# AI-ON/Few-Shot-Music-Generation

Hardware: AMD Instinct MI355X
Metric: episodes/s (LSTM-baseline train step, synthetic vocab=10k seq_len=128 5-way/5-shot h=512) (higher is better)
Workload: dtype f32 (bf16x3-split products, fp32 accumulate)

## Files before the change

### few-shot-music-generation_amd/csrc/api_comm.hip

```cpp
#include "fsmg_model.h"

using namespace fsmg;
using namespace fsmg_host;

namespace fsmg_host {

struct Rccl {
    typedef struct { char internal[128]; } UniqueId;
    int (*GetUniqueId)(UniqueId*) = nullptr;
    int (*CommInitRank)(void**, int, UniqueId, int) = nullptr;
    int (*CommDestroy)(void*) = nullptr;
    int (*AllReduce)(const void*, void*, size_t, int, int, void*, hipStream_t) = nullptr;
    int (*Broadcast)(const void*, void*, size_t, int, int, void*, hipStream_t) = nullptr;
    int (*GroupStart)() = nullptr; int (*GroupEnd)() = nullptr;
    const char* (*GetErrorString)(int) = nullptr;
    std::string why;
    bool ok = false;
    Rccl() {
        static const char* names[] = {"librccl.so", "librccl.so.1", "/opt/rocm/lib/librccl.so.1", "/opt/rocm/lib/librccl.so"};
        void* lib = nullptr;
        for (const char* name : names) if (!lib) lib = dlopen(name, RTLD_NOW | RTLD_NOLOAD | RTLD_GLOBAL);
        for (const char* name : names) if (!lib) lib = dlopen(name, RTLD_NOW | RTLD_GLOBAL);
        if (!lib) { why = "librccl.so not found (dlopen)"; return; }
        GetUniqueId = (int (*)(UniqueId*))dlsym(lib, "ncclGetUniqueId");
        CommInitRank = (int (*)(void**, int, UniqueId, int))dlsym(lib, "ncclCommInitRank");
        CommDestroy = (int (*)(void*))dlsym(lib, "ncclCommDestroy");
        AllReduce = (int (*)(const void*, void*, size_t, int, int, void*, hipStream_t))dlsym(lib, "ncclAllReduce");
        Broadcast = (int (*)(const void*, void*, size_t, int, int, void*, hipStream_t))dlsym(lib, "ncclBroadcast");
        GroupStart = (int (*)())dlsym(lib, "ncclGroupStart");
        GroupEnd = (int (*)())dlsym(lib, "ncclGroupEnd");
        GetErrorString = (const char* (*)(int))dlsym(lib, "ncclGetErrorString");
        ok = GetUniqueId && CommInitRank && CommDestroy && AllReduce && Broadcast && GroupStart && GroupEnd && GetErrorString;
        if (!ok) why = "librccl.so lacks an expected symbol";
    }
};
inline Rccl& rccl() { static Rccl r; return r; }
constexpr int NCCL_FLOAT = 7, NCCL_SUM = 0, NCCL_CHAR = 0;
#define NCCLCK(h, call)                                                                                   \
    do {                                                                                                  \
        const int e_ = (call);                                                                            \
        if (e_ != 0) return fail(h, FSMG_ERR_HIP, std::string(#call) + ": " + rccl().GetErrorString(e_)); \
    } while (0)

void comm_destroy(fsmg_model* h) {
    if (h->comm && h->own_comm && rccl().ok) rccl().CommDestroy(h->comm);
    if (h->ev_comm) hipEventDestroy(h->ev_comm);
    if (h->comm_stream) hipStreamDestroy(h->comm_stream);
    h->comm = nullptr; h->ev_comm = nullptr; h->comm_stream = nullptr;
}

int exchange_gradients(fsmg_model* h) {
    Rccl& r = rccl();
    HIPCK(h, hipStreamWaitEvent(h->comm_stream, h->ev_bucket[0], 0));
    NCCLCK(h, r.AllReduce(h->G + h->off_w, h->G + h->off_w, (size_t)(h->n_flat - h->off_w), NCCL_FLOAT, NCCL_SUM, h->comm, h->comm_stream));
    HIPCK(h, hipStreamWaitEvent(h->comm_stream, h->ev_bucket[1], 0));
    NCCLCK(h, r.GroupStart());
    NCCLCK(h, r.AllReduce(h->G, h->G, (size_t)h->off_w, NCCL_FLOAT, NCCL_SUM, h->comm, h->comm_stream));
    NCCLCK(h, r.AllReduce(h->G + h->n_flat, h->G + h->n_flat, (size_t)FSMG_GRAD_TAIL, NCCL_FLOAT, NCCL_SUM, h->comm, h->comm_stream));
    NCCLCK(h, r.GroupEnd());
    HIPCK(h, hipEventRecord(h->ev_comm, h->comm_stream));
    HIPCK(h, hipStreamWaitEvent(h->stream, h->ev_comm, 0));
    return FSMG_OK;
}

}

extern "C" {

static int comm_prepare(fsmg_handle h) {
    if (!rccl().ok) return fail(h, FSMG_ERR_STATE, "RCCL is not available: " + rccl().why);
    BEGIN_CALL(h);
    if (!h->comm_stream) HIPCK(h, hipStreamCreateWithFlags(&h->comm_stream, hipStreamNonBlocking));
    if (!h->ev_comm) HIPCK(h, hipEventCreateWithFlags(&h->ev_comm, hipEventDisableTiming));
    return FSMG_OK;
}

int fsmg_comm_unique_id(char id[FSMG_COMM_ID_BYTES]) {
    if (!id) return FSMG_ERR_INVALID;
    if (!rccl().ok) return fail(nullptr, FSMG_ERR_STATE, "RCCL is not available: " + rccl().why);
    Rccl::UniqueId u;
    const int e = rccl().GetUniqueId(&u);
    if (e != 0) return fail(nullptr, FSMG_ERR_HIP, std::string("ncclGetUniqueId: ") + rccl().GetErrorString(e));
    std::memcpy(id, u.internal, FSMG_COMM_ID_BYTES);
    return FSMG_OK;
}

int fsmg_comm_init(fsmg_handle h, const char id[FSMG_COMM_ID_BYTES], int32_t world_size, int32_t rank) {
    if (!h || !id || world_size < 1 || rank < 0 || rank >= world_size) return FSMG_ERR_INVALID;
    if (h->comm) return fail(h, FSMG_ERR_STATE, "a communicator is already attached");
    int rc = comm_prepare(h);
    if (rc != FSMG_OK) return rc;
    Rccl::UniqueId u;
    std::memcpy(u.internal, id, FSMG_COMM_ID_BYTES);
    void* c = nullptr;
    NCCLCK(h, rccl().CommInitRank(&c, world_size, u, rank));
    h->comm = c; h->own_comm = true; h->world = world_size; h->rank = rank;
    drop_graphs(h);
    return FSMG_OK;
}

int fsmg_comm_attach(fsmg_handle h, void* nccl_comm, int32_t world_size, int32_t rank) {
    if (!h || !nccl_comm || world_size < 1 || rank < 0 || rank >= world_size) return FSMG_ERR_INVALID;
    if (h->comm) return fail(h, FSMG_ERR_STATE, "a communicator is already attached");
    int rc = comm_prepare(h);
    if (rc != FSMG_OK) return rc;
    h->comm = nccl_comm; h->own_comm = false; h->world = world_size; h->rank = rank;
// ... 32 lines not shown
```

### few-shot-music-generation_amd/csrc/api_debug.hip

```cpp
#include "fsmg_model.h"

using namespace fsmg;
using namespace fsmg_host;


extern "C" {

int fsmg_debug_clock_begin(fsmg_handle h, int32_t microseconds) {
    if (!h || microseconds <= 0 || microseconds > 1000000) return FSMG_ERR_INVALID;
    BEGIN_CALL(h, true);
    if (!h->probe) HIPCK(h, hipStreamCreateWithFlags(&h->probe, hipStreamNonBlocking));
    if (!h->d_probe) HIPCK(h, hipMalloc((void**)&h->d_probe, 64));
    HIPCK(h, hipMemsetAsync(h->d_probe, 0, 64, h->probe));
    HIPCK(h, launch_clock_probe(h->probe, (long long)microseconds * 100, h->d_probe));
    return FSMG_OK;
}
int fsmg_debug_clock_end(fsmg_handle h, float* ghz) {
    if (!h || !ghz) return FSMG_ERR_INVALID;
    if (!h->probe || !h->d_probe) return fail(h, FSMG_ERR_STATE, "fsmg_debug_clock_end without fsmg_debug_clock_begin");
    BEGIN_CALL(h, true);
    unsigned long long v[2] = {0, 0};
    HIPCK(h, hipStreamSynchronize(h->probe));
    HIPCK(h, hipMemcpy(v, h->d_probe, sizeof(v), hipMemcpyDeviceToHost));
    *ghz = v[1] ? (float)((double)v[0] / (double)v[1] * 0.1) : 0.0f;
    return FSMG_OK;
}

int fsmg_debug_dims(fsmg_handle h, int32_t dims[5]) {
    if (!h || !dims) return FSMG_ERR_INVALID;
    dims[0] = h->Ep; dims[1] = h->Hp; dims[2] = h->V1p; dims[3] = h->lastB; dims[4] = h->T;
    return FSMG_OK;
}

int fsmg_debug_read(fsmg_handle h, const char* what, float* host, int64_t count) {
    if (!h || !what || !host || count <= 0) return FSMG_ERR_INVALID;
    const int upd_state = h->upd_deferred ? 2 : h->upd_pending ? 1 : 0;
    BEGIN_CALL(h, !std::strcmp(what, "upd_defer"));
    const int64_t B = h->lastB, T = h->T, Hp = h->Hp, G4 = h->G4, rows = T * B;
    const float* src = nullptr; int64_t cap = 0;
    auto layer_of = [&](const char* prefix) -> int {
        const size_t n = std::strlen(prefix);
        if (std::strncmp(what, prefix, n) != 0) return -1;
        const int l = std::atoi(what + n);
        return (l >= 0 && l < h->L && std::strlen(what) > n) ? l : -1;
    };
    int l;
    if (!std::strcmp(what, "aux_tries")) { host[0] = (float)h->aux_tries; return FSMG_OK; }
    if (!std::strcmp(what, "fused_softmax")) { host[0] = h->fused_softmax ? 1.0f : 0.0f; if (count > 1) host[1] = h->fs_call ? 1.0f : 0.0f; return FSMG_OK; }
    if (!std::strcmp(what, "upd_defer")) {
        const float v[4] = {h->upd_defer ? 1.0f : 0.0f, (float)upd_state, (float)h->n_upd_placed, (float)h->n_upd_settled};
        for (int64_t i = 0; i < count && i < 4; ++i) host[i] = v[i];
        return FSMG_OK;
    }
    if (!std::strcmp(what, "xcd_bx3")) { host[0] = h->xcd_bx3 ? 1.0f : 0.0f; return FSMG_OK; }
    if (!std::strcmp(what, "gemm_kinds")) {
        for (int64_t i = 0; i < count && i < 4; ++i) host[i] = (float)h->gemm_kinds[i];
        return FSMG_OK;
    }
    if (!std::strcmp(what, "xov_selfcheck")) {
        const float v[3] = {(float)h->xov_selfcheck_runs, (float)h->xov_passes, (float)h->xov_selfcheck_every};
        for (int64_t i = 0; i < count && i < 3; ++i) host[i] = v[i];
        return FSMG_OK;
    }
    if (!std::strcmp(what, "xcd_partitioned")) {
        host[0] = h->xov ? 1.0f : 0.0f;
        if (count > 1) { const int b = h->lastB > 0 ? h->lastB : 45, rpx = lstm_xcd16_packed_rows(b, h->Hp); host[1] = (h->xov && rpx > 0) ? (float)xov_first_free(b, h->Hp) : 8.0f; }
        if (count > 2) host[2] = h->xov_last ? 1.0f : 0.0f;
        return FSMG_OK;
    }
    if (!std::strncmp(what, "adapted:", 8)) {
        if (!h->have_adapted) return fail(h, FSMG_ERR_STATE, "no adapted parameters kept: fsmg_debug_set(\"keep_adapted\", 1), then a MAML-style call");
        return download_tensor(h, h->P_adapted, what + 8, host, count);
    }
    if (!std::strcmp(what, "logits")) { src = h->logits; cap = rows * h->V1p; }
    else if (!std::strcmp(what, "dlogits")) { src = dlogits_buf(h); cap = rows * h->V1p; }
    else if (!std::strcmp(what, "lse")) { src = h->lse; cap = rows; }
    else if (!std::strcmp(what, "ce")) { src = h->ce; cap = rows; }
    else if (!std::strcmp(what, "row_weight")) { src = h->roww; cap = h->last_mask_groups > 0 ? rows : 0; }
    else if (!std::strcmp(what, "n_valid")) {
        if (count > h->last_mask_groups) return fail(h, FSMG_ERR_SIZE, "debug read larger than the buffer");
        std::vector<int> nv((size_t)count);
        HIPCK(h, hipStreamSynchronize(h->stream));
        HIPCK(h, hipMemcpy(nv.data(), h->d_nvalid, sizeof(int) * count, hipMemcpyDeviceToHost));
        for (int64_t i = 0; i < count; ++i) host[i] = (float)nv[(size_t)i];
// ... 88 lines not shown
```

### few-shot-music-generation_amd/csrc/api_forward.hip

```cpp
#include "fsmg_model.h"

using namespace fsmg;
using namespace fsmg_host;

namespace fsmg_host {

int stage_tokens(fsmg_model* h, const int32_t* support, int n_sup, const int32_t* query, int n_qry, int on_device) {
    const size_t T = h->T;
    if (on_device && h->eager_call) {
        h->cur_sup = support; h->cur_qry = query;
        return FSMG_OK;
    }
    const hipMemcpyKind kind = on_device ? hipMemcpyDeviceToDevice : hipMemcpyHostToDevice;
    if (n_sup > 0) HIPCK(h, hipMemcpyAsync(h->d_tok, support, sizeof(int) * n_sup * T, kind, h->stream));
    if (n_qry > 0) HIPCK(h, hipMemcpyAsync(h->d_tok + n_sup * T, query, sizeof(int) * n_qry * T, kind, h->stream));
    h->cur_sup = h->d_tok; h->cur_qry = h->d_tok + n_sup * T;
    return FSMG_OK;
}

int stage_lengths(fsmg_model* h, const int32_t* support_len, int n_sup, const int32_t* query_len, int n_qry, int on_device) {
    const hipMemcpyKind kind = on_device ? hipMemcpyDeviceToDevice : hipMemcpyHostToDevice;
    if (n_sup > 0) HIPCK(h, hipMemcpyAsync(h->d_len, support_len, sizeof(int) * n_sup, kind, h->stream));
    if (n_qry > 0) HIPCK(h, hipMemcpyAsync(h->d_len + n_sup, query_len, sizeof(int) * n_qry, kind, h->stream));
    h->cur_len = h->d_len;
// ... 95 lines not shown
}

int forward(fsmg_model* h, int B, int rows_per_group, int ngroups, float* loss_out, bool want_dlogits, int head) {
    ScopedRange rng_(want_dlogits ? "fsmg.forward(train)" : head == HEAD_LOGITS ? "fsmg.forward(score)" : head == HEAD_NONE ? "fsmg.forward(cache)" : "fsmg.forward(eval)");
    const int T = h->T, Hp = h->Hp, G4 = h->G4;
    const int64_t rows = (int64_t)T * B;
    const Lane mainl = main_lane(h);
    hipStream_t s = h->stream;
    const bool ov = head == HEAD_LOSS && use_overlap(h);
    const bool xcd = use_xcd(h, B);
    const bool chain1 = !xcd && h->persist && !h->force_fwd_rt && lstm_fwd_chain_supported(B, Hp);
    const bool chain_rt = !xcd && h->persist && !chain1 && lstm_fwd_chain_rt_supported(B, Hp);
    const bool chain = chain1 || chain_rt;
    if (!xcd && h->cs_stale) return fail(h, FSMG_ERR_STATE, "internal: forward pass on the column-split kernels with stale fragment copies of K_h (ensure_cs not called)");
    const int nch_ov = ov ? ((chain || xcd) ? h->nchunk_persist : h->nchunk) : 1;
    GemmArgs ghead = logits_args(h, B, 0, T);
    h->fs_call = false;
    if (want_dlogits && h->fused_softmax && !ov && h->bx3 && h->inplace_dlogits && h->Hsc != nullptr && mainl.lds_pad == 0) {
        h->fs_call = true;
        h->fs_call = use_h_gemm(h, OP_XC, OP_XC, dw_args(h, B), mainl);
    }
    if (h->fs_call) fused_softmax_args(h, ghead);
    const bool xov = h->xov_call && (h->xov_parts & 1) && xcd && want_dlogits && !ov && xov_fits(ghead);
    const int xfree = xov_first_free(B, Hp);
    const int rpx = xov ? lstm_xcd16_packed_rows(B, Hp) : 0;
    if (xov) xov_gate(h, ghead, B);
    for (int l = 0; l < h->L; ++l) {
        const size_t Bp16 = (size_t)(B + 15) / 16 * 16;
        const bool top = l == h->L - 1;
        FillBatch fills(h);
        GEMMCK(fills.add(h->Hs[l], 0u, (long long)B * Hp));
        GEMMCK(fills.add(h->Cs[l], 0u, (long long)B * Hp));
        if (!xcd) GEMMCK(fills.add(h->HF[l], 0u, (long long)Bp16 * Hp));
        {
            ScopedTimer tm(h, "gemm_zx");
            GemmArgs g{};
            if (l == 0) { g.A = h->P + h->off_emb; g.lda = h->Ep; g.gather = h->X; g.K = h->Ep; }
            else { g.A = h->Hs[l - 1] + (size_t)B * Hp; g.lda = Hp; g.K = Hp; }
            g.B = h->P + h->off_kx[l]; g.ldb = G4;
            g.C = h->Z[l]; g.ldc = G4; g.M = (int)rows; g.N = G4;
            g.bias = h->P + h->off_b[l]; g.ksplit = 1;
            GEMMCK(gemm(h, mainl, OP_KC, OP_XC, g));
        }
        auto chain_fills = [&]() -> int {
            if (chain)
                GEMMCK(fills.add(h->HF[l] + Bp16 * Hp, 0xFFFFFFFFu, (long long)T * Bp16 * Hp));
            if (xcd) {
                GEMMCK(fills.add(h->tickets, 0u, (long long)8 * fsmg_model::TICKET_LAUNCHES));
                h->ticket_next = 0;
                const int rpx_l = xov && top ? rpx : 0;
                const long long step_f = lstm_xcd_hx_floats(B, 0, Hp, h->xcd_bx3, rpx_l);
                const long long used_f = step_f / lstm_xcd_slices(Hp) * lstm_xcd_used_slices(B, rpx_l, Hp);
                GEMMCK(fills.add(h->HX, 0u, step_f));
                GEMMCK(fills.add_strided(h->HX + step_f, 0xFFFFFFFFu, used_f, step_f, T));
                if (xov && top) {
                    GEMMCK(fills.add(h->xov_ctl, 0u, 4 + gemm_items(ghead)));
                    GEMMCK(fills.add(h->xov_prog, 0u, T));
                }
            }
            return fills.flush();
        };
        const bool place = l == 0 && h->upd_deferred && xov && top && xfree >= 1 && xfree <= 7;
        if (place) GEMMCK(place_deferred_half(h, xfree));
        GEMMCK(chain_fills());
        if (l == 0 && !place) GEMMCK(settle_pending(h));
        if (xov && top) {
            HIPCK(h, hipEventRecord(h->ev_fork, s));
            HIPCK(h, hipStreamWaitEvent(h->aux, h->ev_fork, 0));
            GEMMCK(gemm_restricted(h, h->aux, OP_KC, OP_XC, ghead, xfree, h->xov_ctl));
            HIPCK(h, hipEventRecord(h->ev_join, h->aux));
        }
        const int nch = nch_ov;
        for (int c = 0; c < nch; ++c) {
            const int t0 = chunk_begin(h, c, nch);
            const int t1 = chunk_begin(h, c + 1, nch);
            if (xcd) {
                ScopedTimer tm(h, "lstm_fwd");
                LstmFwdXcdArgs a{};
                a.rpx = (xov && top) ? rpx : 0; a.progress = (xov && top) ? h->xov_prog : nullptr; a.Hp = Hp;
                a.progress_every = h->xov_pub; a.bx3 = h->xcd_bx3 ? 1 : 0;
                a.variant = h->xcd_variant >= 0 ? h->xcd_variant : lstm_xcd_default_variant(B, true, Hp, a.rpx, h->xcd_bx3);
                a.KhX = h->khx + (size_t)(2 * l) * lstm_xcd_weight_floats((int)Hp, h->xcd_bx3); a.HX = h->HX; a.Z = h->Z[l]; a.Cs = h->Cs[l]; a.Hs = h->Hs[l];
                a.tickets = next_tickets(h); a.err_flag = h->d_err; a.B = B; a.T = T; a.t0 = t0; a.t1 = t1; a.spin_limit = h->chain_spin_limit;
                HIPCK(h, launch_lstm_fwd_xcd(s, a));
                ++h->n_xcd_launches;
            } else if (chain) {
                ScopedTimer tm(h, "lstm_fwd");
                LstmFwdChainArgs a{};
                a.KhF = h->khf + (size_t)(2 * l) * Hp * G4; a.HF = h->HF[l]; a.Z = h->Z[l]; a.Cs = h->Cs[l]; a.Hs = h->Hs[l];
                a.err_flag = h->d_err; a.B = B; a.Hp = Hp; a.T = T; a.t0 = t0; a.t1 = t1; a.spin_limit = h->chain_spin_limit;
                HIPCK(h, chain_rt ? launch_lstm_fwd_chain_rt(s, a) : launch_lstm_fwd_chain(s, a));
                ++h->n_persist_launches;
            } else {
                ScopedTimer tm(h, "lstm_fwd");
                for (int t = t0; t < t1; ++t) {
                    LstmFwdArgs a{};
                    a.KhF = h->khf + (size_t)(2 * l) * Hp * G4;
                    a.hF_prev = h->HF[l] + (size_t)t * Bp16 * Hp;
                    a.hF_next = h->HF[l] + (size_t)(t + 1) * Bp16 * Hp;
                    a.z = h->Z[l] + (size_t)t * B * G4;
                    a.c_prev = h->Cs[l] + (size_t)t * B * Hp;
// ... 59 lines not shown
```

### few-shot-music-generation_amd/csrc/api_handle.hip

```cpp
#include <mutex>
#include "fsmg_model.h"

using namespace fsmg;
using namespace fsmg_host;

namespace fsmg_host {

thread_local std::string g_create_error;

static int pick_concurrent_aux(fsmg_model* h, int priority, int max_tries) {
    if (max_tries <= 0) {
        if (hipStreamCreateWithPriority(&h->aux, hipStreamNonBlocking, priority) != hipSuccess) return fail(h, FSMG_ERR_HIP, "aux stream create failed");
        h->aux_tries = 0;
        return FSMG_OK;
    }
    int* d = nullptr;
    if (hipMalloc((void**)&d, 256) != hipSuccess) return fail(h, FSMG_ERR_NOMEM, "hipMalloc(queue probe) failed");
    auto probe = [&](hipStream_t cand, long long ticks) -> int {
        int seen = 0;
        const int init[2] = {0, -1};
        if (hipStreamSynchronize(h->stream) != hipSuccess || hipMemcpy(d, init, sizeof(init), hipMemcpyHostToDevice) != hipSuccess ||
            launch_queue_probe(h->stream, d, d + 1, 0, ticks) != hipSuccess || launch_queue_probe(cand, d, d + 1, 1, 0) != hipSuccess ||
            hipStreamSynchronize(cand) != hipSuccess || hipStreamSynchronize(h->stream) != hipSuccess ||
            hipMemcpy(&seen, d + 1, sizeof(int), hipMemcpyDeviceToHost) != hipSuccess) return -1;
// ... 7 lines not shown
        const int seen = probe(cand, 30000);
        if (seen < 0) { hipStreamDestroy(cand); rc = fail(h, FSMG_ERR_HIP, "queue probe failed"); break; }
        if (seen == 1) { h->aux = cand; h->aux_tries = t; found = 1; }
        else rejected.push_back(cand);
    }
    for (size_t i = 0; rc == FSMG_OK && !found && i < rejected.size(); ++i) {
        const int seen = probe(rejected[i], 500000);
        if (seen < 0) { rc = fail(h, FSMG_ERR_HIP, "queue probe failed"); break; }
        if (seen == 1) { h->aux = rejected[i]; h->aux_tries = (int)(max_tries + i + 1); found = 1; rejected.erase(rejected.begin() + (long)i); }
    }
    if (rc == FSMG_OK && !found) {
        h->aux = rejected.back(); rejected.pop_back();
        h->aux_tries = -1;
    }
    for (hipStream_t s : rejected) hipStreamDestroy(s);
    hipFree(d);
    return rc;
}

int settle_pending(fsmg_model* h) {
    if (h->upd_deferred) {
        h->upd_deferred = false;
        UpdateArgs b = h->upd_half;
        b.xcd_first = 0; b.chunk_ctr = nullptr;
        HIPCK(h, launch_adam_update(h->stream, b));
        ++h->n_upd_settled;
    }
    if (!h->upd_pending) return FSMG_OK;
    h->upd_pending = false;
    HIPCK(h, hipStreamWaitEvent(h->stream, h->ev_upd, 0));
    return FSMG_OK;
}

int place_deferred_half(fsmg_model* h, int xcd_first) {
    if (!h->upd_deferred) return FSMG_OK;
    if (h->aux == nullptr || h->d_upd_ctr == nullptr || !h->upd_ctr_zeroed || xcd_first < 1 || xcd_first > 7) return settle_pending(h);
    h->upd_deferred = false;
    h->upd_ctr_zeroed = false;
    UpdateArgs b = h->upd_half;
    b.xcd_first = xcd_first; b.chunk_ctr = h->d_upd_ctr;
    HIPCK(h, hipEventRecord(h->ev_upd_fork, h->stream));
    HIPCK(h, hipStreamWaitEvent(h->aux, h->ev_upd_fork, 0));
    HIPCK(h, launch_adam_update(h->aux, b));
    HIPCK(h, hipEventRecord(h->ev_upd, h->aux));
    h->upd_pending = true;
    ++h->n_upd_placed;
    return FSMG_OK;
}

std::mutex& turn_mutex() { static std::mutex mu; return mu; }
namespace {
fsmg_model* g_turn_last[16] = {};
bool turnstile_on() { static const bool on = !(std::getenv("FSMG_TURNSTILE") && std::atoi(std::getenv("FSMG_TURNSTILE")) == 0); return on; }
}
static int take_turn(fsmg_model* h) {
    if (!turnstile_on() || h->ev_turn == nullptr) return FSMG_OK;
    std::lock_guard<std::mutex> lk(turn_mutex());
    fsmg_model*& last = g_turn_last[h->device & 15];
    auto capturing = [](hipStream_t s) {
        hipStreamCaptureStatus st = hipStreamCaptureStatusNone;
        return s != nullptr && hipStreamIsCapturing(s, &st) == hipSuccess && st != hipStreamCaptureStatusNone;
    };
    if (last != nullptr && last != h && last->stream != nullptr && !last->capturing.load() && !capturing(last->stream) && !capturing(last->aux)) {
        HIPCK(h, hipEventRecord(last->ev_turn, last->stream));
        HIPCK(h, hipEventRecord(last->ev_turn_aux, last->aux != nullptr ? last->aux : last->stream));
        HIPCK(h, hipStreamWaitEvent(h->stream, last->ev_turn, 0));
        HIPCK(h, hipStreamWaitEvent(h->stream, last->ev_turn_aux, 0));
        if (h->aux != nullptr) {
            HIPCK(h, hipStreamWaitEvent(h->aux, last->ev_turn, 0));
            HIPCK(h, hipStreamWaitEvent(h->aux, last->ev_turn_aux, 0));
        }
    }
    last = h;
    return FSMG_OK;
}
// ... 47 lines not shown
    h->device = cfg->device;
    compute_dims(*cfg, h);
    h->n_flat = build_layout(h);
    auto bail = [&](int code, const std::string& msg) { g_create_error = msg; fsmg_destroy(h); return code; };

    if (cfg->stream) { h->stream = (hipStream_t)cfg->stream; h->own_stream = false; }
    else {
        if (hipStreamCreateWithFlags(&h->stream, hipStreamNonBlocking) != hipSuccess) return bail(FSMG_ERR_HIP, "hipStreamCreate failed");
        h->own_stream = true;
    }
    {
        if (const char* eg = std::getenv("FSMG_GRAPH")) h->cfg.use_graph = (eg[0] != '0');
        h->overlap = (int64_t)h->V1 >= 8LL * h->H * h->L;
        if (cfg->schedule == FSMG_SCHEDULE_SINGLE_STREAM) { h->overlap = false; h->overlap_forced = true; }
        if (cfg->schedule == FSMG_SCHEDULE_TWO_STREAM) { h->overlap = true; h->overlap_forced = true; }
        if (cfg->schedule == FSMG_SCHEDULE_XCD_PARTITIONED) h->xov = true;
        if (cfg->gemm == FSMG_GEMM_F32) h->bx3 = 0;
        if (cfg->recurrence == FSMG_RECURRENCE_PER_STEP) h->persist = false;
        if (cfg->recurrence == FSMG_RECURRENCE_COLUMN_SPLIT) h->xcd = false;
        if (cfg->recurrence == FSMG_RECURRENCE_XCD_LOCAL) h->pair_mode = 2;
        if (cfg->dp_split_backward) h->dp_split = cfg->dp_split_backward == 2 ? 2 : 1;
        const char* env = std::getenv("FSMG_OVERLAP");
        if (env) { h->overlap = env[0] != '0'; h->overlap_forced = true; }
        if (const char* e = std::getenv("FSMG_GEMM")) h->bx3 = std::strcmp(e, "f32") != 0;
        if (const char* e = std::getenv("FSMG_GEMM_H")) h->gemm_h = std::atoi(e);
        if (const char* e = std::getenv("FSMG_GEMM_WS")) h->gemm_ws = std::atoi(e);
        if (const char* e = std::getenv("FSMG_MAX_SPLIT")) h->max_split = std::max(1, std::atoi(e));
        if (const char* e = std::getenv("FSMG_XCD_OVERLAP")) h->xov = std::atoi(e) != 0;
        if (const char* e = std::getenv("FSMG_XOV_PARTS")) h->xov_parts = std::max(1, std::min(7, std::atoi(e)));
        if (const char* e = std::getenv("FSMG_EAGER")) h->eager = (e[0] != '0');
        if (const char* e = std::getenv("FSMG_MERGE_DK")) h->merge_dk = (e[0] != '0');
        if (const char* e = std::getenv("FSMG_UPD_SPLIT")) h->upd_split = (e[0] != '0');
        if (const char* e = std::getenv("FSMG_UPD_DEFER")) h->upd_defer = (e[0] != '0');
        if (const char* e = std::getenv("FSMG_TAIL_ASIDE")) h->tail_aside = (e[0] != '0');
        if (const char* e = std::getenv("FSMG_LAZY_CS")) h->lazy_cs = (e[0] != '0');
        if (const char* e = std::getenv("FSMG_FUSED_SOFTMAX")) h->fused_softmax = (e[0] != '0');

        if (const char* e = std::getenv("FSMG_INPLACE_DLOGITS")) h->inplace_dlogits = (e[0] != '0');
        if (const char* e = std::getenv("FSMG_XOV_SELFCHECK")) h->xov_selfcheck_left = std::max(0, std::atoi(e));
        if (const char* e = std::getenv("FSMG_XOV_SELFCHECK_EVERY")) h->xov_selfcheck_every = std::max(0, std::atoi(e));
        if (const char* e = std::getenv("FSMG_PERSISTENT")) h->persist = (e[0] != '0');
        h->persist_cfg = h->persist;
        if (const char* e = std::getenv("FSMG_FALLBACK_STEPS")) h->fallback_steps = std::max(1, std::atoi(e));
        if (const char* e = std::getenv("FSMG_XCD")) h->xcd = (e[0] != '0');
        if (const char* e = std::getenv("FSMG_XCD_PAIR")) h->pair_mode = std::max(0, std::min(2, std::atoi(e)));
        if (const char* e = std::getenv("FSMG_FWD_RT")) h->force_fwd_rt = (e[0] != '0');
        if (const char* e = std::getenv("FSMG_CHAIN_SPIN_LIMIT")) h->chain_spin_limit = std::max(0, std::atoi(e));
        if (const char* e = std::getenv("FSMG_XCD_VARIANT")) h->xcd_variant = std::atoi(e);
        if (const char* e = std::getenv("FSMG_XCD_VARIANT_BWD")) h->xcd_variant_bwd = std::atoi(e);
        if (hipEventCreateWithFlags(&h->ev_turn, hipEventDisableTiming) != hipSuccess ||
            hipEventCreateWithFlags(&h->ev_turn_aux, hipEventDisableTiming) != hipSuccess) return bail(FSMG_ERR_HIP, "event create failed");
        if (turnstile_on()) {
            std::lock_guard<std::mutex> lk(turn_mutex());
            fsmg_model* last = g_turn_last[h->device & 15];
            if (last != nullptr && last->stream != nullptr && !last->capturing.load()) { (void)hipStreamSynchronize(last->stream); if (last->aux) (void)hipStreamSynchronize(last->aux); }
        }
        {
            static const int tries = std::getenv("FSMG_AUX_TRIES") ? std::max(0, std::min(32, std::atoi(std::getenv("FSMG_AUX_TRIES")))) : 8;
            if (pick_concurrent_aux(h, 0, tries) != FSMG_OK) { std::string e = h->err; return bail(FSMG_ERR_HIP, e); }
            if (h->aux_tries < 0) {
                fprintf(stderr, "[fsmg] no second stream of this process runs beside the handle's stream (%d candidates, probed for 300 us and again for 5 ms: "
                                "they share its hardware queue -- GPU_MAX_HW_QUEUES? -- or the device was busy with another process): serial order, no overlapped "
                                "tails for this handle (fsmg_stats.aux_stream_tries = -1; fsmg_debug_set(\"reprobe_aux\", 1) asks again)\n", tries);
                h->overlap = false; h->overlap_forced = true; h->tail_aside = false; h->upd_split = false;
            }
        }
        for (int c = 0; c < fsmg_model::NCHUNK; ++c)
            if (hipEventCreateWithFlags(&h->ev_chunk[c], hipEventDisableTiming) != hipSuccess) return bail(FSMG_ERR_HIP, "event create failed");
        if (hipEventCreateWithFlags(&h->ev_bucket[0], hipEventDisableTiming) != hipSuccess ||
            hipEventCreateWithFlags(&h->ev_bucket[1], hipEventDisableTiming) != hipSuccess ||
            hipEventCreateWithFlags(&h->ev_fork, hipEventDisableTiming) != hipSuccess ||
            hipEventCreateWithFlags(&h->ev_upd_fork, hipEventDisableTiming) != hipSuccess ||
            hipEventCreateWithFlags(&h->ev_upd, hipEventDisableTiming) != hipSuccess ||
            hipEventCreateWithFlags(&h->ev_side_fork, hipEventDisableTiming) != hipSuccess ||
            hipEventCreateWithFlags(&h->ev_side, hipEventDisableTiming) != hipSuccess ||

            hipEventCreateWithFlags(&h->ev_join, hipEventDisableTiming) != hipSuccess) return bail(FSMG_ERR_HIP, "event create failed");
    }
    const int64_t sb = state_bytes_for(h->n_flat);
    if (cfg->state_arena) {
        if (cfg->state_arena_bytes < (uint64_t)sb || ((uintptr_t)cfg->state_arena & 255u))
            return bail(FSMG_ERR_INVALID, "state_arena too small or not 256-byte aligned");
        h->state = (char*)cfg->state_arena; h->own_state = false;
    } else {
        if (hipMalloc((void**)&h->state, sb) != hipSuccess) return bail(FSMG_ERR_NOMEM, "hipMalloc(state) failed");
        h->own_state = true;
    }
    h->P = (float*)h->state; h->G = h->P + h->n_flat;
    h->M = h->G + h->n_flat + FSMG_GRAD_TAIL; h->Vv = h->M + h->n_flat;
    if (hipMemsetAsync(h->state, 0, sb, h->stream) != hipSuccess) return bail(FSMG_ERR_HIP, "memset(state) failed");

    char* small = nullptr;
    const size_t tok_words = (size_t)round_up(h->V1, 64);
    const size_t prog_words = (size_t)round_up(h->T + 8, 64);
    const size_t small_bytes = 256 * 4 + sizeof(float) * RING_CAP + sizeof(int) * 8 * fsmg_model::TICKET_LAUNCHES + sizeof(int) * 2 * fsmg_model::XOV_CTL +
                               sizeof(int) * 2 * tok_words + sizeof(int) * prog_words;
    if (hipMalloc((void**)&small, small_bytes) != hipSuccess) return bail(FSMG_ERR_NOMEM, "hipMalloc(scalars) failed");
    hipMemsetAsync(small, 0, small_bytes, h->stream);
    h->d_step = (long long*)small; h->d_err = (int*)(small + 256); h->d_gnorm = (float*)(small + 512);
    h->d_inbox_dirty = (int*)(small + 768);
    h->d_decided = (float*)(small + 896);
    h->d_upd_ctr = (int*)(small + 960);
    { static const int one = 1; hipStreamSynchronize(h->stream); hipMemcpy(h->d_inbox_dirty, &one, sizeof(int), hipMemcpyHostToDevice); }
    h->d_ring = (float*)(small + 1024);
    if (hipHostMalloc((void**)&h->host_counters, 64, hipHostMallocMapped) != hipSuccess ||
        hipHostGetDevicePointer((void**)&h->d_counters, h->host_counters, 0) != hipSuccess)
        return bail(FSMG_ERR_NOMEM, "hipHostMalloc(mapped step counters) failed");
    std::memset(h->host_counters, 0, 64);
    h->tickets = (int*)(small + 1024 + sizeof(float) * RING_CAP);
    h->xov_ctl = h->tickets + 8 * fsmg_model::TICKET_LAUNCHES;
// ... 99 lines not shown
    if (!h || !out) return FSMG_ERR_INVALID;
    BEGIN_CALL(h);
    HIPCK(h, hipStreamSynchronize(h->stream));
    poll_skipped(h);
    std::memset(out, 0, sizeof(*out));
    out->timeouts = h->n_timeouts;
    out->steps_skipped_timeout = h->host_counters ? h->host_counters[0] : 0;
    out->steps_skipped_token_range = h->host_counters ? h->host_counters[1] : 0;
    out->steps_skipped_peer_failure = h->host_counters ? h->host_counters[2] : 0;
    out->xov_selfcheck_mismatches = h->host_counters ? h->host_counters[3] : 0;
    out->softmax_range_rows = h->host_counters ? h->host_counters[4] : 0;
    out->steps_skipped_softmax_range = h->host_counters ? h->host_counters[5] : 0;
    out->aux_stream_tries = h->aux_tries; out->reserved0 = 0;
    out->xcd_launches = h->n_xcd_launches;
    out->persistent_launches = h->n_persist_launches;
    out->step_launches = h->n_step_launches;
    out->persistent_path = h->persist ? 1 : 0;
    out->fallback_steps_left = h->fallback_left;
    return FSMG_OK;
}

int fsmg_debug_set(fsmg_handle h, const char* what, int64_t value) {
    if (!h || !what) return FSMG_ERR_INVALID;
    BEGIN_CALL(h);
    HIPCK(h, hipStreamSynchronize(h->stream));
    if (h->aux) HIPCK(h, hipStreamSynchronize(h->aux));
    if (!std::strcmp(what, "chain_spin_limit")) h->chain_spin_limit = (int)std::max<int64_t>(0, std::min<int64_t>(value, 1 << 30));
    else if (!std::strcmp(what, "fallback_steps")) h->fallback_steps = (int)std::max<int64_t>(1, std::min<int64_t>(value, 1 << 30));
    else if (!std::strcmp(what, "eager")) h->eager = value != 0;
    else if (!std::strcmp(what, "persistent")) { h->persist = h->persist_cfg = value != 0; h->fallback_left = 0; }
    else if (!std::strcmp(what, "inplace_dlogits")) h->inplace_dlogits = value != 0;
    else if (!std::strcmp(what, "upd_split")) h->upd_split = value != 0;
    else if (!std::strcmp(what, "upd_defer")) h->upd_defer = value != 0;
    else if (!std::strcmp(what, "reprobe_aux")) {
        if (value != 0 && h->aux_tries < 0) {
            HIPCK(h, hipStreamSynchronize(h->stream));
            if (h->aux) HIPCK(h, hipStreamSynchronize(h->aux));
            hipStream_t old = h->aux; h->aux = nullptr;
            const int rc = pick_concurrent_aux(h, 0, 8);
            if (rc != FSMG_OK) { if (h->aux == nullptr) h->aux = old; return rc; }
            if (old) hipStreamDestroy(old);
            if (h->aux_tries > 0) {
                h->overlap = true; h->overlap_forced = false; h->tail_aside = true;
                if (h->xov_eligible && h->xcd_bx3) h->xov = true;
                drop_graphs(h);
            }
        }
    }
    else if (!std::strcmp(what, "tail_aside")) h->tail_aside = value != 0;
    else if (!std::strcmp(what, "fused_softmax")) h->fused_softmax = value != 0;
    else if (!std::strcmp(what, "keep_adapted")) h->keep_adapted = value != 0;
    else if (!std::strcmp(what, "xov_selfcheck")) h->xov_selfcheck_left = (int)std::max<int64_t>(0, std::min<int64_t>(value, 1 << 30));
    else if (!std::strcmp(what, "xov_selfcheck_fault")) h->xov_selfcheck_fault = value != 0;
    else if (!std::strcmp(what, "xov_selfcheck_every")) h->xov_selfcheck_every = (int)std::max<int64_t>(0, std::min<int64_t>(value, 1 << 30));
    else return fail(h, FSMG_ERR_NAME, std::string("unknown knob '") + what + "'");
    drop_graphs(h);
    return FSMG_OK;
}

}
```

### few-shot-music-generation_amd/csrc/fsmg_model.h

```cpp
#pragma once
#include <atomic>
#include <hip/hip_runtime.h>
#include <dlfcn.h>

#include <algorithm>
#include <cmath>
#include <cstdlib>
#include <new>
#include <cstdio>
#include <cstring>
#include <functional>
#include <map>
#include <mutex>
#include <string>
#include <vector>

#include "../../include/fsmg.h"
#include "fsmg_kernels.h"

namespace fsmg_host {
using namespace fsmg;
struct OpBatch;

inline int64_t round_up(int64_t x, int64_t m) { return (x + m - 1) / m * m; }
// ... 117 lines not shown
    bool xcd_bx3 = false;
    bool xcd_bx3_forced = false;
    float* HX = nullptr; int64_t hx_floats = 0;
    float* inboxX = nullptr; int64_t inboxx_floats = 0;
    int* d_inbox_dirty = nullptr;
    int* tickets = nullptr;
    static constexpr int TICKET_LAUNCHES = 64;
    int ticket_next = 0;
    int64_t n_timeouts = 0, n_persist_launches = 0, n_xcd_launches = 0, n_step_launches = 0;
    bool khf_dirty = true;
    bool lazy_cs = true;
    bool cs_stale = false;
    float* slabs = nullptr;
    float* arena = nullptr;
    int64_t arena_cap = 0, arena_off = 0;
    bool warned_split = false;
    int* tok_first = nullptr; int* tok_count = nullptr;
    bool tok_table_open = false;
    bool last_bwd_xcd = false;
    bool eager = true, eager_call = false;
    const int* cur_sup = nullptr; const int* cur_qry = nullptr;
    float* colsum_slabs = nullptr;
    float* slabs2 = nullptr;
    float* colsum_slabs2 = nullptr;
    hipStream_t probe = nullptr;
    unsigned long long* d_probe = nullptr;
    hipStream_t aux = nullptr;
    int aux_tries = 0;
    static constexpr int NCHUNK = 16;
    static constexpr int nchunk = 8;
    static constexpr int nchunk_persist = 4;
    static constexpr int aux_blocks_persist = 2;
    static constexpr int aux_blocks_per_cu = 2;
    hipEvent_t ev_chunk[NCHUNK] = {};
    hipEvent_t ev_fork = nullptr, ev_join = nullptr;
    bool merge_dk = true;
    hipEvent_t ev_bucket[2] = {};
    bool overlap = true;
    bool overlap_forced = false;
    bool ov_call = false;
    int bx3 = 1;
    int gemm_h = 1;
    int gemm_ws = 1;
    int max_split = fsmg_host::MAX_SPLIT;
    long long gemm_kinds[4] = {};
    bool xov = false, xov_call = false;
    bool xov_eligible = false;
    bool bucket0_recorded = false;
    static constexpr int xov_dw_split = 4;
    static constexpr int xov_pub = 6;
    int xov_strikes = 0;
    bool xov_last = false;
    int xov_parts = 3;
    int* xov_prog = nullptr;
    static constexpr int XOV_CTL = 8192;
    int* xov_ctl = nullptr;
    int64_t slab_cap = 0;
    std::map<std::string, hipGraphExec_t> graphs;
    struct LaunchCounts { int64_t xcd = 0, persist = 0, step = 0; bool bwd_xcd = false; };
    std::map<std::string, LaunchCounts> graph_counts;
    char* gen = nullptr;
    size_t gen_bytes = 0;
    std::vector<fsmg_dstate_s*> dstates;
    std::vector<fsmg_cache_s*> caches;
    char* cat = nullptr;
    size_t cat_bytes = 0;

    void* comm = nullptr; bool own_comm = false; int world = 1, rank = 0;
    hipStream_t comm_stream = nullptr;
    hipEvent_t ev_comm = nullptr;
    int lastB = 0;
    bool have_grads = false;
    bool upd_split = false;
    bool upd_pending = false;
    hipEvent_t ev_upd_fork = nullptr, ev_upd = nullptr;
    float* d_decided = nullptr;
    bool upd_defer = true;
    bool upd_deferred = false;
    fsmg::UpdateArgs upd_half{};
    int* d_upd_ctr = nullptr;
    bool upd_ctr_zeroed = false;
    long long n_upd_placed = 0, n_upd_settled = 0;
    fsmg_host::OpBatch* slabs_owner = nullptr;
    int xov_selfcheck_left = 2;
    int xov_selfcheck_every = 1000;
    long long xov_passes = 0, xov_selfcheck_runs = 0;
    bool xov_selfcheck_fault = false;
    long long seen_selfcheck_mismatch = 0;
    bool inplace_dlogits = true;
    bool fused_softmax = true;
    bool fs_call = false;
    float* Hsc = nullptr;
    float* crow = nullptr;
    long long seen_softmax_range = 0;
    bool tail_aside = true;
    bool side_pending = false;
    hipEvent_t ev_side_fork = nullptr, ev_side = nullptr;
    hipEvent_t ev_turn = nullptr, ev_turn_aux = nullptr;
    std::atomic<bool> capturing{false};
    std::string err;
    bool timing = false;
    std::string timing_only;
    std::map<std::string, fsmg_host::TimerClass> timers;
};

namespace fsmg_host {

extern thread_local std::string g_create_error;
// ... 221 lines not shown
}

inline int* next_tickets(fsmg_model* h) {
    int* t = h->tickets + 8 * (h->ticket_next % fsmg_model::TICKET_LAUNCHES);
    ++h->ticket_next;
    return t;
}

inline int gemm_items(const GemmArgs& g) { return ((g.M + 255) / 256) * ((g.N + 255) / 256) * std::max(1, g.ksplit); }
inline bool xov_fits(const GemmArgs& g) { return 4 + gemm_items(g) <= fsmg_model::XOV_CTL; }
void choose_schedule(fsmg_model* h, int B, bool train = false);
void xov_gate(fsmg_model* h, GemmArgs& g, int B);
int gemm_prepare_queue(fsmg_model* h, GemmArgs& g, int split, OpBatch* defer, bool* ok);
int select_xcd_format(fsmg_model* h, int B);
int gemm_restricted(fsmg_model* h, hipStream_t s, int amode, int bmode, GemmArgs g, int first, int* ctl);
int gemm_cleanup(fsmg_model* h, hipStream_t s, int amode, int bmode, GemmArgs g, int* ctl);

int stage_tokens(fsmg_model* h, const int32_t* support, int n_sup, const int32_t* query, int n_qry, int on_device);
int reset_tok_table(fsmg_model* h);
int token_prep(fsmg_model* h, int n_sup, int n_qry, bool train = false);
int stage_lengths(fsmg_model* h, const int32_t* support_len, int n_sup, const int32_t* query_len, int n_qry, int on_device);
enum { HEAD_LOSS = 0, HEAD_LOGITS = 1, HEAD_NONE = 2 };
int forward(fsmg_model* h, int B, int rows_per_group, int ngroups, float* loss_out, bool want_dlogits, int head = HEAD_LOSS);
GemmArgs dw_args(fsmg_model* h, int B);
int backward(fsmg_model* h, int B, int part = 0);
int repack_recurrent_weights(fsmg_model* h, hipStream_t s, const StepIncArgs* inc, bool* inc_done);
int repack_recurrent_weights(fsmg_model* h, hipStream_t s);
int ensure_khf(fsmg_model* h);
int ensure_cs(fsmg_model* h);
inline bool pass_reads_cs(const fsmg_model* h, int B, bool train) {
    return !use_xcd(h, B) || (train && !use_xcd(h, B, true));
}
int apply_update(fsmg_model* h, float grad_scale, bool may_defer = false);
int place_deferred_half(fsmg_model* h, int xcd_first);
int sgd_update(fsmg_model* h, float lr);
int save_theta(fsmg_model* h);
int restore_theta(fsmg_model* h);
int keep_theta_prime(fsmg_model* h);
void on_timeout(fsmg_model* h);
void on_softmax_range(fsmg_model* h);
inline bool is_retry(int rc) { return rc == FSMG_ERR_TIMEOUT || rc == FSMG_ERR_SOFTMAX_RANGE; }
int with_adapted_theta(fsmg_model* h, const int32_t* support, int32_t n_support_rows, int32_t inner_steps, float inner_lr,
                       int32_t support_on_device, const std::function<int()>& at_theta_prime);
int poll_skipped(fsmg_model* h);
int report(fsmg_model* h, int what);
int check_tokens_and_read(fsmg_model* h, const float* d_src, float scale, float* host_out, int n, bool train_tail = false);
int after_update(fsmg_model* h, float grad_scale, float* loss);
int run_passes(fsmg_model* h, const int32_t* tokens, int R, int P, int on_device, const std::function<int(int, int)>& launch,
               const std::function<int(int, int)>& read_back);
int check_host_tokens(fsmg_model* h, const int32_t* tokens, size_t n);
void row_nll(const float* logprob, int R, int T, int nll_first, int nll_count, float* out);
void row_nll_masked(const float* logprob, int R, int T, int nll_first, int nll_count, const int32_t* len, float* out);
int check_host_lengths(fsmg_model* h, const int32_t* len, size_t n);
int gen_reserve(fsmg_model* h, size_t bytes);
fsmg_cache_s* find_cache(fsmg_model* h, fsmg_cache c);
struct CacheGen {
    const fsmg_cache_s* c = nullptr;
    float theta = 0.f, lambda = 0.f;
    int R = 0, ldl = 0;
    std::vector<int> slot_query, tile_group, row_group;
    int *d_slot_query = nullptr, *d_tile_group = nullptr, *d_row_group = nullptr;
    double* D = nullptr;
    float* pc = nullptr;
    int W = 0, NP = 0, ldo = 0, Hp = 0;
    bool raw = false;
    float* own_keys = nullptr;
    double* D2 = nullptr;
// ... 18 lines not shown
```

Before: 649.0.

## Issue head fills before zx GEMM and create stream-seam events without system fence

Reorders the layer-0 forward so the chain fills (when head_fills_first is on, the default) go out before the input GEMM. The deferred Adam half-update is now launched on the aux stream behind the existing head fork, which saves a separate fork event. Inter-stream seam events are now created with hipEventDisableSystemFence to make event record and wait cheaper. A debug readout of event flags is also added. The reordering changes when work overlaps on the aux stream and could delay the zx GEMM. Dropping the system fence assumes no host-visible coherence is needed at these seams.

```diff
diff --git a/few-shot-music-generation_amd/csrc/api_comm.hip b/few-shot-music-generation_amd/csrc/api_comm.hip
--- a/few-shot-music-generation_amd/csrc/api_comm.hip
+++ b/few-shot-music-generation_amd/csrc/api_comm.hip
@@ -46,7 +46,7 @@
     if (h->comm && h->own_comm && rccl().ok) rccl().CommDestroy(h->comm);
     if (h->ev_comm) hipEventDestroy(h->ev_comm);
     if (h->comm_stream) hipStreamDestroy(h->comm_stream);
-    h->comm = nullptr; h->ev_comm = nullptr; h->comm_stream = nullptr;
+    h->comm = nullptr; h->ev_comm = nullptr; h->ev_flags[fsmg_model::EVF_COMM] = 0; h->comm_stream = nullptr;
 }
 
 int exchange_gradients(fsmg_model* h) {
@@ -71,7 +71,7 @@
     if (!rccl().ok) return fail(h, FSMG_ERR_STATE, "RCCL is not available: " + rccl().why);
     BEGIN_CALL(h);
     if (!h->comm_stream) HIPCK(h, hipStreamCreateWithFlags(&h->comm_stream, hipStreamNonBlocking));
-    if (!h->ev_comm) HIPCK(h, hipEventCreateWithFlags(&h->ev_comm, hipEventDisableTiming));
+    if (!h->ev_comm) { HIPCK(h, hipEventCreateWithFlags(&h->ev_comm, hipEventDisableTiming)); h->ev_flags[fsmg_model::EVF_COMM] = hipEventDisableTiming | fsmg_model::EVF_CREATED; }
     return FSMG_OK;
 }
 
diff --git a/few-shot-music-generation_amd/csrc/api_debug.hip b/few-shot-music-generation_amd/csrc/api_debug.hip
--- a/few-shot-music-generation_amd/csrc/api_debug.hip
+++ b/few-shot-music-generation_amd/csrc/api_debug.hip
@@ -35,7 +35,7 @@
 int fsmg_debug_read(fsmg_handle h, const char* what, float* host, int64_t count) {
     if (!h || !what || !host || count <= 0) return FSMG_ERR_INVALID;
     const int upd_state = h->upd_deferred ? 2 : h->upd_pending ? 1 : 0;
-    BEGIN_CALL(h, !std::strcmp(what, "upd_defer"));
+    BEGIN_CALL(h, !std::strcmp(what, "upd_defer") || !std::strcmp(what, "event_flags"));
     const int64_t B = h->lastB, T = h->T, Hp = h->Hp, G4 = h->G4, rows = T * B;
     const float* src = nullptr; int64_t cap = 0;
     auto layer_of = [&](const char* prefix) -> int {
@@ -50,6 +50,14 @@
     if (!std::strcmp(what, "upd_defer")) {
         const float v[4] = {h->upd_defer ? 1.0f : 0.0f, (float)upd_state, (float)h->n_upd_placed, (float)h->n_upd_settled};
         for (int64_t i = 0; i < count && i < 4; ++i) host[i] = v[i];
+        return FSMG_OK;
+    }
+    if (!std::strcmp(what, "event_flags")) {
+        for (int64_t i = 0; i < count && i < fsmg_model::EVF_N; ++i) {
+            const unsigned f = h->ev_flags[i];
+            host[i] = !(f & fsmg_model::EVF_CREATED) ? -1.0f : (float)(((f & hipEventDisableTiming) ? 1 : 0) + ((f & hipEventDisableSystemFence) ? 2 : 0) + ((f & hipEventReleaseToDevice) ? 4 : 0) +
+                                                 ((f & hipEventReleaseToSystem) ? 8 : 0) + ((f & hipEventBlockingSync) ? 16 : 0) + ((f & hipEventInterprocess) ? 32 : 0));
+        }
         return FSMG_OK;
     }
     if (!std::strcmp(what, "xcd_bx3")) { host[0] = h->xcd_bx3 ? 1.0f : 0.0f; return FSMG_OK; }
diff --git a/few-shot-music-generation_amd/csrc/api_forward.hip b/few-shot-music-generation_amd/csrc/api_forward.hip
--- a/few-shot-music-generation_amd/csrc/api_forward.hip
+++ b/few-shot-music-generation_amd/csrc/api_forward.hip
@@ -151,7 +151,7 @@
         GEMMCK(fills.add(h->Hs[l], 0u, (long long)B * Hp));
         GEMMCK(fills.add(h->Cs[l], 0u, (long long)B * Hp));
         if (!xcd) GEMMCK(fills.add(h->HF[l], 0u, (long long)Bp16 * Hp));
-        {
+        auto zx_gemm = [&]() -> int {
             ScopedTimer tm(h, "gemm_zx");
             GemmArgs g{};
             if (l == 0) { g.A = h->P + h->off_emb; g.lda = h->Ep; g.gather = h->X; g.K = h->Ep; }
@@ -160,7 +160,8 @@
             g.C = h->Z[l]; g.ldc = G4; g.M = (int)rows; g.N = G4;
             g.bias = h->P + h->off_b[l]; g.ksplit = 1;
             GEMMCK(gemm(h, mainl, OP_KC, OP_XC, g));
-        }
+            return FSMG_OK;
+        };
         auto chain_fills = [&]() -> int {
             if (chain)
                 GEMMCK(fills.add(h->HF[l] + Bp16 * Hp, 0xFFFFFFFFu, (long long)T * Bp16 * Hp));
@@ -179,13 +180,17 @@
             }
             return fills.flush();
         };
-        const bool place = l == 0 && h->upd_deferred && xov && top && xfree >= 1 && xfree <= 7;
-        if (place) GEMMCK(place_deferred_half(h, xfree));
-        GEMMCK(chain_fills());
+        const bool fills_first = xov && top && h->head_fills_first;
+        if (fills_first) GEMMCK(chain_fills());
+        GEMMCK(zx_gemm());
+        const bool place = l == 0 && h->upd_deferred && xov && top && xfree >= 1 && xfree <= 7 && upd_half_placeable(h);
+        if (place && !fills_first) GEMMCK(place_deferred_half(h, xfree, false));
+        if (!fills_first) GEMMCK(chain_fills());
         if (l == 0 && !place) GEMMCK(settle_pending(h));
         if (xov && top) {
             HIPCK(h, hipEventRecord(h->ev_fork, s));
             HIPCK(h, hipStreamWaitEvent(h->aux, h->ev_fork, 0));
+            if (place && fills_first) GEMMCK(place_deferred_half(h, xfree, true));
             GEMMCK(gemm_restricted(h, h->aux, OP_KC, OP_XC, ghead, xfree, h->xov_ctl));
             HIPCK(h, hipEventRecord(h->ev_join, h->aux));
         }
diff --git a/few-shot-music-generation_amd/csrc/api_handle.hip b/few-shot-music-generation_amd/csrc/api_handle.hip
--- a/few-shot-music-generation_amd/csrc/api_handle.hip
+++ b/few-shot-music-generation_amd/csrc/api_handle.hip
@@ -63,15 +63,18 @@
     return FSMG_OK;
 }
 
-int place_deferred_half(fsmg_model* h, int xcd_first) {
+bool upd_half_placeable(const fsmg_model* h) { return h->aux != nullptr && h->d_upd_ctr != nullptr && h->upd_ctr_zeroed; }
+int place_deferred_half(fsmg_model* h, int xcd_first, bool forked) {
     if (!h->upd_deferred) return FSMG_OK;
-    if (h->aux == nullptr || h->d_upd_ctr == nullptr || !h->upd_ctr_zeroed || xcd_first < 1 || xcd_first > 7) return settle_pending(h);
+    if (!upd_half_placeable(h) || xcd_first < 1 || xcd_first > 7) return forked ? fail(h, FSMG_ERR_STATE, "internal: deferred half cannot be placed behind the fork") : settle_pending(h);
     h->upd_deferred = false;
     h->upd_ctr_zeroed = false;
     UpdateArgs b = h->upd_half;
     b.xcd_first = xcd_first; b.chunk_ctr = h->d_upd_ctr;
-    HIPCK(h, hipEventRecord(h->ev_upd_fork, h->stream));
-    HIPCK(h, hipStreamWaitEvent(h->aux, h->ev_upd_fork, 0));
+    if (!forked) {
+        HIPCK(h, hipEventRecord(h->ev_upd_fork, h->stream));
+        HIPCK(h, hipStreamWaitEvent(h->aux, h->ev_upd_fork, 0));
+    }
     HIPCK(h, launch_adam_update(h->aux, b));
     HIPCK(h, hipEventRecord(h->ev_upd, h->aux));
     h->upd_pending = true;
@@ -185,6 +188,7 @@
         if (const char* e = std::getenv("FSMG_MERGE_DK")) h->merge_dk = (e[0] != '0');
         if (const char* e = std::getenv("FSMG_UPD_SPLIT")) h->upd_split = (e[0] != '0');
         if (const char* e = std::getenv("FSMG_UPD_DEFER")) h->upd_defer = (e[0] != '0');
+        if (const char* e = std::getenv("FSMG_HEAD_FILLS_FIRST")) h->head_fills_first = (e[0] != '0');
         if (const char* e = std::getenv("FSMG_TAIL_ASIDE")) h->tail_aside = (e[0] != '0');
         if (const char* e = std::getenv("FSMG_LAZY_CS")) h->lazy_cs = (e[0] != '0');
         if (const char* e = std::getenv("FSMG_FUSED_SOFTMAX")) h->fused_softmax = (e[0] != '0');
@@ -201,8 +205,9 @@
         if (const char* e = std::getenv("FSMG_CHAIN_SPIN_LIMIT")) h->chain_spin_limit = std::max(0, std::atoi(e));
         if (const char* e = std::getenv("FSMG_XCD_VARIANT")) h->xcd_variant = std::atoi(e);
         if (const char* e = std::getenv("FSMG_XCD_VARIANT_BWD")) h->xcd_variant_bwd = std::atoi(e);
-        if (hipEventCreateWithFlags(&h->ev_turn, hipEventDisableTiming) != hipSuccess ||
-            hipEventCreateWithFlags(&h->ev_turn_aux, hipEventDisableTiming) != hipSuccess) return bail(FSMG_ERR_HIP, "event create failed");
+        auto new_event = [&](hipEvent_t* e, unsigned flags, int slot) { h->ev_flags[slot] = flags | fsmg_model::EVF_CREATED; return hipEventCreateWithFlags(e, flags); };
+        if (new_event(&h->ev_turn, hipEventDisableTiming, fsmg_model::EVF_TURN) != hipSuccess ||
+            new_event(&h->ev_turn_aux, hipEventDisableTiming, fsmg_model::EVF_TURN_AUX) != hipSuccess) return bail(FSMG_ERR_HIP, "event create failed");
         if (turnstile_on()) {
             std::lock_guard<std::mutex> lk(turn_mutex());
             fsmg_model* last = g_turn_last[h->device & 15];
@@ -219,16 +224,15 @@
             }
         }
         for (int c = 0; c < fsmg_model::NCHUNK; ++c)
-            if (hipEventCreateWithFlags(&h->ev_chunk[c], hipEventDisableTiming) != hipSuccess) return bail(FSMG_ERR_HIP, "event create failed");
-        if (hipEventCreateWithFlags(&h->ev_bucket[0], hipEventDisableTiming) != hipSuccess ||
-            hipEventCreateWithFlags(&h->ev_bucket[1], hipEventDisableTiming) != hipSuccess ||
-            hipEventCreateWithFlags(&h->ev_fork, hipEventDisableTiming) != hipSuccess ||
-            hipEventCreateWithFlags(&h->ev_upd_fork, hipEventDisableTiming) != hipSuccess ||
-            hipEventCreateWithFlags(&h->ev_upd, hipEventDisableTiming) != hipSuccess ||
-            hipEventCreateWithFlags(&h->ev_side_fork, hipEventDisableTiming) != hipSuccess ||
-            hipEventCreateWithFlags(&h->ev_side, hipEventDisableTiming) != hipSuccess ||
-
-            hipEventCreateWithFlags(&h->ev_join, hipEventDisableTiming) != hipSuccess) return bail(FSMG_ERR_HIP, "event create failed");
+            if (new_event(&h->ev_chunk[c], fsmg_model::SEAM_EVENT_FLAGS, fsmg_model::EVF_CHUNK + c) != hipSuccess) return bail(FSMG_ERR_HIP, "event create failed");
+        if (new_event(&h->ev_bucket[0], hipEventDisableTiming, fsmg_model::EVF_BUCKET0) != hipSuccess ||
+            new_event(&h->ev_bucket[1], hipEventDisableTiming, fsmg_model::EVF_BUCKET1) != hipSuccess ||
+            new_event(&h->ev_fork, fsmg_model::SEAM_EVENT_FLAGS, fsmg_model::EVF_FORK) != hipSuccess ||
+            new_event(&h->ev_upd_fork, fsmg_model::SEAM_EVENT_FLAGS, fsmg_model::EVF_UPD_FORK) != hipSuccess ||
+            new_event(&h->ev_upd, fsmg_model::SEAM_EVENT_FLAGS, fsmg_model::EVF_UPD) != hipSuccess ||
+            new_event(&h->ev_side_fork, fsmg_model::SEAM_EVENT_FLAGS, fsmg_model::EVF_SIDE_FORK) != hipSuccess ||
+            new_event(&h->ev_side, fsmg_model::SEAM_EVENT_FLAGS, fsmg_model::EVF_SIDE) != hipSuccess ||
+            new_event(&h->ev_join, fsmg_model::SEAM_EVENT_FLAGS, fsmg_model::EVF_JOIN) != hipSuccess) return bail(FSMG_ERR_HIP, "event create failed");
     }
     const int64_t sb = state_bytes_for(h->n_flat);
     if (cfg->state_arena) {
@@ -394,6 +398,7 @@
     else if (!std::strcmp(what, "inplace_dlogits")) h->inplace_dlogits = value != 0;
     else if (!std::strcmp(what, "upd_split")) h->upd_split = value != 0;
     else if (!std::strcmp(what, "upd_defer")) h->upd_defer = value != 0;
+    else if (!std::strcmp(what, "head_fills_first")) h->head_fills_first = value != 0;
     else if (!std::strcmp(what, "reprobe_aux")) {
         if (value != 0 && h->aux_tries < 0) {
             HIPCK(h, hipStreamSynchronize(h->stream));
diff --git a/few-shot-music-generation_amd/csrc/fsmg_model.h b/few-shot-music-generation_amd/csrc/fsmg_model.h
--- a/few-shot-music-generation_amd/csrc/fsmg_model.h
+++ b/few-shot-music-generation_amd/csrc/fsmg_model.h
@@ -173,6 +173,10 @@
     static constexpr int nchunk_persist = 4;
     static constexpr int aux_blocks_persist = 2;
     static constexpr int aux_blocks_per_cu = 2;
+    static constexpr unsigned SEAM_EVENT_FLAGS = hipEventDisableTiming | hipEventDisableSystemFence;
+    enum { EVF_BUCKET0, EVF_BUCKET1, EVF_TURN, EVF_TURN_AUX, EVF_COMM, EVF_FORK, EVF_JOIN, EVF_UPD_FORK, EVF_UPD, EVF_SIDE_FORK, EVF_SIDE, EVF_CHUNK, EVF_N = EVF_CHUNK + NCHUNK };
+    static constexpr unsigned EVF_CREATED = 0x100;
+    unsigned ev_flags[EVF_N] = {};
     hipEvent_t ev_chunk[NCHUNK] = {};
     hipEvent_t ev_fork = nullptr, ev_join = nullptr;
     bool merge_dk = true;
@@ -215,6 +219,7 @@
     bool upd_split = false;
     bool upd_pending = false;
     hipEvent_t ev_upd_fork = nullptr, ev_upd = nullptr;
+    bool head_fills_first = true;
     float* d_decided = nullptr;
     bool upd_defer = true;
     bool upd_deferred = false;
@@ -502,7 +507,8 @@
     return !use_xcd(h, B) || (train && !use_xcd(h, B, true));
 }
 int apply_update(fsmg_model* h, float grad_scale, bool may_defer = false);
-int place_deferred_half(fsmg_model* h, int xcd_first);
+bool upd_half_placeable(const fsmg_model* h);
+int place_deferred_half(fsmg_model* h, int xcd_first, bool forked);
 int sgd_update(fsmg_model* h, float lr);
 int save_theta(fsmg_model* h);
 int restore_theta(fsmg_model* h);
```

After: 652.4 (median of 6 runs). No clear change (+0.5%).
